# dhillon24/3d-shape-generation

Hardware: AMD Instinct MI355X
Metric: denoising-steps/sec (whole node), 2048-pt DDPM, batch 64 (higher is better)
Workload: dtype f16; 1 GPU; BASELINE configs[1]: point-cloud DDPM (sample2), 2048 points, batch 64 per GPU, 1000-step cosine schedule, fp16 operands/fp32 accumulate, random-init synthetic weights, denoiser UNetPointNetLarge; batch_per_gpu=64, points=2048, sampler=ddpm/sample2, backbone=pointnet, launch=eager, rccl_ranks=1

## Files before the change

### 3d-shape-generation_amd/_lib.py

```python
from __future__ import annotations

import ctypes as C
import os
import subprocess
from typing import Optional

_HERE = os.path.dirname(os.path.abspath(__file__))
LIB_PATH = os.path.join(_HERE, "libpcd_hip.so")
ABI_VERSION = 2
CSRC = os.path.join(_HERE, "csrc")

vp = C.c_void_p
i32, i64, u64, f32, sz = C.c_int, C.c_int64, C.c_uint64, C.c_float, C.c_size_t

PCD_UNET_NLIN = 26


class GemmDesc(C.Structure):
    _fields_ = [("a1", vp), ("lda1", i64), ("k1", i32),
                ("a2", vp), ("lda2", i64), ("k2", i32),
                ("w", vp), ("ldw", i64),
                ("bias", vp), ("shape_bias", vp), ("rows_per_shape", i32),
                ("relu", i32), ("m", i32), ("c", i32)]

# ... 141 lines not shown
    "pcd_head3": (i32, [vp, i64, i32, vp, vp, vp, vp]),
    "pcd_pw_chain_enc1": (i32, [vp, i64, i32, vp, vp, i32, vp, vp, vp, vp, vp, vp]),
    "pcd_pw_chain_enc1_hilo": (i32, [vp, i64, i32, vp, vp, i32, vp, vp, vp, vp, vp, vp]),
    "pcd_pw_chain_tail_hilo": (i32, [vp, i64, vp, vp, vp, vp, vp, vp, vp, vp, vp, vp]),
    "pcd_pw_chain_128": (i32, [vp, i64, vp, vp, vp, vp, vp, vp]),
    "pcd_pw_chain_tail": (i32, [vp, i64, vp, vp, vp, vp, vp, vp, vp, vp, vp, vp]),
    "pcd_unet_config": (i32, [i32]),
    "pcd_panel_chain": (i32, [i32, vp, i64, vp, vp, i32, vp, i64, i32, vp]),
    "pcd_panel_chain_dec": (i32, [vp, vp, i64, vp, vp, i32, vp, i64, i32, vp]),
    "pcd_pw_wide_packed_bytes": (sz, [i32]),
    "pcd_pw_wide_pack": (i32, [i32, vp, vp, vp, vp]),
    "pcd_pw_wide_chain": (i32, [i32, vp, vp, i64, vp, vp, vp]),
    "pcd_pw_wide_ends_packed_bytes": (sz, [i32, i32]),
    "pcd_pw_wide_ends_pack": (i32, [i32, i32, vp, vp, vp, vp]),
    "pcd_pw_wide_ends": (i32, [i32, i32, vp, vp, vp, i64, vp, vp, vp, vp]),
    "pcd_conv1x1_supported": (i32, [i32, i32]),
    "pcd_conv1x1_f16": (i32, [vp, i64, i32, vp, i64, vp, i32, i32, vp, vp]),
    "pcd_unet_create": (i32, [C.POINTER(UnetDesc), C.POINTER(vp)]),
    "pcd_unet_destroy": (None, [vp]),
    "pcd_unet_workspace_bytes": (sz, [i32, i32]),
    "pcd_unet_forward": (i32, [vp, vp, i32, i32, vp, i32, vp, vp, sz, vp]),
    "pcd_unet_profile": (i32, [vp, i32]),
    "pcd_unet_profile_read": (i32, [vp, C.POINTER(C.c_double), C.POINTER(i32)]),
    "pcd_unet_tap": (i32, [vp, C.c_char_p, i32, i32, vp, vp, sz, vp]),
    "pcd_unet_capture": (i32, [vp, vp, vp, vp, vp]),
    "pcd_gemm_f32": (i32, [vp, i64, i32, vp, i64, i32, vp, i64, vp, vp, i32, i32, i32, i32, vp, i64, vp]),
    "pcd_gemm_f32_colmax": (i32, [vp, i64, i32, vp, i64, vp, i32, i32, vp, i32, vp]),
    "pcd_unet_f32_create": (i32, [C.POINTER(UnetDesc), C.POINTER(vp)]),
    "pcd_unet_f32_destroy": (None, [vp]),
    "pcd_unet_f32_workspace_bytes": (sz, [i32, i32]),
# ... 253 lines not shown
```

### 3d-shape-generation_amd/csrc/stage_images.h

```cpp
#pragma once
#include "common.h"

namespace pcd {

static __global__ __launch_bounds__(256) void stage_pack_kernel(const half_t* __restrict__ w, int64_t ldw, int row0, int row_limit, int k0, int ntile, int nq,
                                                                char* __restrict__ dst) {
    const int id = blockIdx.x * blockDim.x + threadIdx.x;
    if (id >= ntile * nq * 64) return;
    const int lane = id & 63, tq = id >> 6, t = tq / nq, q = tq - t * nq;
    const int row = row0 + 32 * t + (lane & 31);
    half8 v;
#pragma unroll
    for (int e = 0; e < 8; ++e) v[e] = (half_t)0.f;
    if (row < row_limit) v = *(const half8*)(w + (int64_t)row * ldw + k0 + 16 * q + 8 * (lane >> 5));
    *(half8*)(dst + (size_t)id * 16) = v;
}

struct FragBlock { int w, ldw, row0, row_limit, k0, ntile, nq, nimg; size_t off; };
struct ParamRow { int src, src_off, n, off; };
struct StageLayout {
    int nblock, nrow;
    size_t par;
    size_t bytes;
    FragBlock block[20];
    ParamRow row[8];
};
constexpr void sl_frag(StageLayout& L, int w, int ldw, int row0, int row_limit, int k0, int ntile, int nq, int nimg = 1) {
    L.block[L.nblock++] = FragBlock{w, ldw, row0, row_limit, k0, ntile, nq, nimg, L.bytes};
    L.bytes += (size_t)nimg * ntile * nq * 1024;
    L.par = L.bytes;
}
constexpr void sl_row(StageLayout& L, int src, int src_off, int n, int width) {
    L.row[L.nrow++] = ParamRow{src, src_off, n, (int)((L.bytes - L.par) / sizeof(float))};
    L.bytes += width * sizeof(float);
}

static inline int stage_pack(const StageLayout& L, const void* const* weights, const float* const* params, void* packed, hipStream_t s) {
    char* dst = (char*)packed;
    PCD_CHECK_HIP(hipMemsetAsync(dst, 0, L.bytes, s));
    for (int i = 0; i < L.nblock; ++i) {
// ... 34 lines not shown
```

### 3d-shape-generation_amd/csrc/unet.hip

```cpp
#include <string.h>
#include <new>
#include "common.h"

struct pcd_unet {
    pcd_unet_desc_t d;
    static constexpr int kMaxEv = 4096;
    int prof_on = 0;
    int prof_n = 0;
    hipEvent_t ev0[kMaxEv];
    hipEvent_t ev1[kMaxEv];
    int ev_created = 0;
    void* wide[2] = {nullptr, nullptr};
    void* ends[2] = {nullptr, nullptr};
    void* gf3_frag = nullptr;
    void* lin_frag[PCD_UNET_NLIN] = {};
    void* dec_tap[4] = {nullptr, nullptr, nullptr, nullptr};
};

namespace pcd {

int pw_chain_enc1_impl(const float* x, int64_t m, int rows_per_shape, const float* w_xyz, const float* tbias, int tbias_shape_stride,
                       const void* w_conv2, const float* b_conv2, const void* w_conv3, const float* b_conv3, void* x1, bool hilo,
                       float* zero, int64_t zero_n, void* stream);


struct UnetWs {
    size_t x1, x2, x3, x4, s0, s1, pooled, pooled16, gbias, total;
};
// ... 16 lines not shown
    return w;
}

}

using namespace pcd;

static const int kLinK[PCD_UNET_NLIN] = {64, 64, 128, 128, 128, 256, 256, 256, 512, 512, 512, 1024, 2048,
                                         1024, 1024, 1024, 1024, 512, 512, 512, 256, 256, 256, 128, 128, 64};
static const int kLinC[PCD_UNET_NLIN] = {64, 128, 128, 128, 256, 256, 256, 512, 512, 512, 1024, 2048, 4096,
                                         1024, 1024, 512, 512, 512, 256, 256, 256, 128, 128, 128, 64, 64};

static int g_unet_chains = 3;

extern "C" int pcd_unet_config(int use_chains) {
    g_unet_chains = use_chains & 15;
    return PCD_OK;
}

extern "C" int pcd_unet_create(const pcd_unet_desc_t* desc, pcd_unet_t** out) {
    PCD_CHECK_ARG(desc != nullptr && out != nullptr);
    PCD_CHECK_ARG(desc->freqs && desc->tw0 && desc->tb0 && desc->tw2 && desc->tb2);
    PCD_CHECK_ARG(desc->e1w_xyz && desc->e1w_t && desc->e1b && desc->wg && desc->head_w && desc->head_b);
    PCD_CHECK_ARG(desc->wg_k == 4096 && desc->wg_c == 1024);
    if (desc->hilo_mask & ~PCD_UNET_HILO_ALLOWED) {
        set_error("pcd_unet_create: hilo_mask 0x%x names layers outside 0x%x", desc->hilo_mask, PCD_UNET_HILO_ALLOWED);
        return PCD_ERR_ARG;
    }
    for (int i = 0; i < PCD_UNET_NLIN; ++i) {
        if (desc->lin[i].w == nullptr || desc->lin[i].b == nullptr || desc->lin[i].k != kLinK[i] ||
            desc->lin[i].c != kLinC[i]) {
// ... 20 lines not shown
    }
    h->gf3_frag = pcd_packed_copy(desc->lin[12].w, (size_t)4096 * 2048 * 2,
                                  [&](void* buf) { return pcd_gemm_pack_wfrag(desc->lin[12].w, 2048, 2048, 4096, buf, nullptr); });
    for (int i = 8; i <= 18; ++i) {
        if (i == 12 || ((desc->hilo_mask >> i) & 1u) || kLinK[i] < 384 || kLinC[i] % 256 != 0) continue;
        h->lin_frag[i] = pcd_packed_copy(desc->lin[i].w, (size_t)kLinK[i] * kLinC[i] * 2,
                                         [&](void* buf) { return pcd_gemm_pack_wfrag(desc->lin[i].w, kLinK[i], kLinK[i], kLinC[i], buf, nullptr); });
    }
    for (int c = 0; c < 2; ++c) {
        const int first = c == 0 ? 2 : 19, nl = c == 0 ? 6 : 4;
        const int hilo = (int)((desc->hilo_mask >> (c == 0 ? 4 : 22)) & 1u);
        const void* w[6]; const float* b[6];
        for (int i = 0; i < nl; ++i) { w[i] = desc->lin[first + i].w; b[i] = desc->lin[first + i].b; }
        h->ends[c] = pcd_packed_copy(w[0], pcd_pw_wide_ends_packed_bytes(c, hilo), [&](void* buf) { return pcd_pw_wide_ends_pack(c, hilo, w, b, buf, nullptr); });
    }
    *out = h;
    return PCD_OK;
}

extern "C" void pcd_unet_destroy(pcd_unet_t* h) {
    if (h == nullptr) return;
    if (h->gf3_frag) (void)hipFree(h->gf3_frag);
    for (int i = 0; i < PCD_UNET_NLIN; ++i) if (h->lin_frag[i]) (void)hipFree(h->lin_frag[i]);
    for (int k = 0; k < 2; ++k) if (h->wide[k]) (void)hipFree(h->wide[k]);
    for (int k = 0; k < 2; ++k) if (h->ends[k]) (void)hipFree(h->ends[k]);
    for (int i = 0; i < h->ev_created; ++i) { (void)hipEventDestroy(h->ev0[i]); (void)hipEventDestroy(h->ev1[i]); }
    delete h;
}

extern "C" int pcd_unet_profile(pcd_unet_t* h, int enable) {
    PCD_CHECK_ARG(h != nullptr);
    h->prof_on = enable ? 1 : 0;
    h->prof_n = 0;
    return PCD_OK;
}

extern "C" int pcd_unet_profile_read(pcd_unet_t* h, double* total_ms, int* launches) {
    PCD_CHECK_ARG(h && total_ms && launches);
    double tot = 0.0;
    for (int i = 0; i < h->prof_n; ++i) {
// ... 45 lines not shown
        set_error("pcd_unet_forward: workspace %zu < required %zu", workspace_bytes, w.total);
        return PCD_ERR_WORKSPACE;
    }
    char* ws = (char*)workspace;
    void *x1 = ws + w.x1, *x2 = ws + w.x2, *x3 = ws + w.x3, *x4 = ws + w.x4, *s0 = ws + w.s0, *s1 = ws + w.s1;
    float* pooled = (float*)(ws + w.pooled);
    float* gbias = (float*)(ws + w.gbias);
    hipStream_t s = (hipStream_t)stream;
    const pcd_unet_desc_t& d = h->d;
    int rc;
    const bool chains = (g_unet_chains & 1) != 0;
    bool pooled_cleared = false;
    const bool wide = (g_unet_chains & 2) != 0 && m % 256 == 0;
    const bool e23 = wide && h->ends[0] != nullptr;
    const bool d21 = wide && h->ends[1] != nullptr && h->dec_tap[2] == nullptr;
    if (chains) {
        const unsigned e1 = d.hilo_mask & 3u;
        if (e1 == 3u || e1 == 0u) {
            PCD_RUN(pw_chain_enc1_impl(x, m, n_points, d.e1w_xyz, tbias, tbias_shape_stride, d.lin[0].w, d.lin[0].b, d.lin[1].w, d.lin[1].b, x1,
                                   e1 == 3u, pooled, (int64_t)batch * 4096, s));
            pooled_cleared = true;
        } else {
            PCD_RUN(pcd_enc1_xyz(x, m, n_points, d.e1w_xyz, 64, tbias, tbias_shape_stride, s0, s));
            PCD_RUN(run_lin(d, 0, m, s0, nullptr, 0, nullptr, 0, s1, s));
            PCD_RUN(run_lin(d, 1, m, s1, nullptr, 0, nullptr, 0, x1, s));
        }
        if (!e23) PCD_RUN(pcd_pw_chain_128(x1, m, d.lin[2].w, d.lin[2].b, d.lin[3].w, d.lin[3].b, s1, s));
    } else {
        PCD_RUN(pcd_enc1_xyz(x, m, n_points, d.e1w_xyz, 64, tbias, tbias_shape_stride, s0, s));
        PCD_RUN(run_lin(d, 0, m, s0, nullptr, 0, nullptr, 0, s1, s));
        PCD_RUN(run_lin(d, 1, m, s1, nullptr, 0, nullptr, 0, x1, s));
        if (!e23) {
            PCD_RUN(run_lin(d, 2, m, x1, nullptr, 0, nullptr, 0, s0, s));
            PCD_RUN(run_lin(d, 3, m, s0, nullptr, 0, nullptr, 0, s1, s));
        }
    }
    if (e23) {
        PCD_RUN(pcd_pw_wide_ends(0, (int)((d.hilo_mask >> 4) & 1u), x1, nullptr, nullptr, m, h->ends[0], x3, x2, s));
    } else {
        PCD_RUN(run_lin(d, 4, m, s1, nullptr, 0, nullptr, 0, x2, s));
        if (wide) {
            PCD_RUN(pcd_pw_wide_chain(0, x2, nullptr, m, h->wide[0], x3, s));
        } else {
            PCD_RUN(run_lin(d, 5, m, x2, nullptr, 0, nullptr, 0, s0, s));
            PCD_RUN(run_lin(d, 6, m, s0, nullptr, 0, nullptr, 0, s1, s));
            PCD_RUN(run_lin(d, 7, m, s1, nullptr, 0, nullptr, 0, x3, s));
        }
    }
    const bool panel = (g_unet_chains & 6) == 2 && m % 128 == 0;
    auto panel_chain = [&](int chain, int first, int nl, const void* in, void* out, int ld) {
        const void* frag[3]; const float* bias[3];
        for (int i = 0; i < nl; ++i) { frag[i] = h->lin_frag[first + i]; bias[i] = d.lin[first + i].b; }
// ... 56 lines not shown
        void* t = s0; s0 = s1; s1 = t;
    } else {
        PCD_RUN(run_lin(d, 15, m, s0, nullptr, 0, nullptr, 0, s1, s, h->lin_frag[15]));
        TAP(0, s1, 512);
        PCD_RUN(run_lin(d, 16, m, s1, x3, 512, nullptr, 0, s0, s, h->lin_frag[16]));
        if (panel && has_frags(17, 2)) {
            PCD_RUN(panel_chain(1, 17, 2, s0, s1, 256));
            void* t = s0; s0 = s1; s1 = t;
        } else {
            PCD_RUN(run_lin(d, 17, m, s0, nullptr, 0, nullptr, 0, s1, s, h->lin_frag[17]));
            PCD_RUN(run_lin(d, 18, m, s1, nullptr, 0, nullptr, 0, s0, s, h->lin_frag[18]));
        }
    }
    TAP(1, s0, 256);
    void *ta = s0, *tb = s1;
    if (d21) {
        PCD_RUN(pcd_pw_wide_ends(1, (int)((d.hilo_mask >> 22) & 1u), s0, x2, x1, m, h->ends[1], s1, nullptr, s));
        ta = s1; tb = s0;
    } else {
        if (wide) {
            PCD_RUN(pcd_pw_wide_chain(1, s0, x2, m, h->wide[1], s1, s));
        } else {
            PCD_RUN(run_lin(d, 19, m, s0, x2, 256, nullptr, 0, s1, s));
            PCD_RUN(run_lin(d, 20, m, s1, nullptr, 0, nullptr, 0, s0, s));
            PCD_RUN(run_lin(d, 21, m, s0, nullptr, 0, nullptr, 0, s1, s));
        }
        TAP(2, s1, 128);
        PCD_RUN(run_lin(d, 22, m, s1, x1, 128, nullptr, 0, s0, s));
    }
    const unsigned tl = (d.hilo_mask >> 23) & 7u;
// ... 36 lines not shown
```

### 3d-shape-generation_amd/csrc/widechain.hip

```cpp
#include "common.h"
#include "stage_images.h"

namespace pcd {

constexpr int WC_WAVES = 8, WC_THREADS = 64 * WC_WAVES, WC_TILE = 32 * WC_WAVES;
constexpr int WC_STAGE = 32768, WC_RING = 3;
constexpr int WC_MAXSEG = 8;

struct WcSeg {
    int src;
    int cont;
    int finish;
    int coff;
    int cvalid;
    int bias_off;
    int keep_b;
    int linear;
};

struct WcParams {
    const half_t* in1; const half_t* in2;
    const char* wpacked;
    const float* bias;
    const float* ln;
// ... 88 lines not shown
    for (const auto& p : pass[chain]) sl_frag(L, p[0], p[1], p[2], p[3], p[4], 8, 4, 4);
    for (const auto& p : pass[chain]) sl_row(L, p[0], p[2], p[5], 256);
    return L;
}
constexpr StageLayout WC_LAYOUT[2] = {wc_layout(0), wc_layout(1)};

constexpr StageLayout wl_layout(int passes) {
    StageLayout L{};
    for (int i = 0; i < passes; ++i) sl_frag(L, 0, 256, 256 * i, 256 * passes, 0, 8, 4, 4);
    sl_row(L, 0, 0, 256 * passes, 256 * passes);
    for (int i = 1; i < 3; ++i) sl_row(L, i, 0, 256, 256);
    return L;
}
constexpr StageLayout WL_LAYOUT[4] = {wl_layout(1), wl_layout(2), wl_layout(3), wl_layout(4)};

constexpr int WE_MAXSEG = 8;
enum { WE_K128_C128 = 0, WE_K128_C256 = 1, WE_K256_C128 = 2, WE_K256_C256 = 3 };

struct WeSeg {
    int kind;
    int src;
    int cont;
    int finish;
    int coff;
    int bias_off;
};

struct WeSegSrc { int layer; int ldw; int c0; int k0; };
struct WePlan {
    int nseg, nstage, nbias, nlayer;
    WeSeg seg[WE_MAXSEG];
    WeSegSrc from[WE_MAXSEG];
    int layer_c[6], layer_bias[6];
};
constexpr int we_kind_images(int kind) { return kind == WE_K128_C128 ? 1 : (kind == WE_K256_C256 ? 4 : 2); }
constexpr void we_add(WePlan& P, int kind, int src, int cont, int finish, int coff, int layer, int ldw, int c0, int k0) {
    P.seg[P.nseg] = WeSeg{kind, src, cont, finish, coff, P.layer_bias[layer] + c0};
    P.from[P.nseg] = WeSegSrc{layer, ldw, c0, k0};
    P.nstage += we_kind_images(kind);
    ++P.nseg;
}
constexpr WePlan we_plan(int chain, int hilo) {
    WePlan P{};
    if (chain == 0) {
        const int c[6] = {128, 128, 256, 256, 256, 512};
        P.nlayer = 6;
        for (int i = 0; i < 6; ++i) { P.layer_c[i] = c[i]; P.layer_bias[i] = P.nbias; P.nbias += c[i]; }
        we_add(P, WE_K128_C128, 1, 0, 1, 0, 0, 128, 0, 0);
        we_add(P, WE_K128_C128, 0, 0, 1, 0, 1, 128, 0, 0);
        if (hilo) {
            we_add(P, WE_K128_C256, 0, 0, 0, 0, 2, 256, 0, 0);
            we_add(P, WE_K128_C256, 0, 1, 3, 0, 2, 256, 0, 128);
        } else {
            we_add(P, WE_K128_C256, 0, 0, 3, 0, 2, 128, 0, 0);
        }
        we_add(P, WE_K256_C256, 0, 0, 1, 0, 3, 256, 0, 0);
        we_add(P, WE_K256_C256, 0, 0, 1, 0, 4, 256, 0, 0);
        we_add(P, WE_K256_C256, 0, 0, 2, 0, 5, 256, 0, 0);
        we_add(P, WE_K256_C256, 0, 0, 2, 256, 5, 256, 256, 0);
    } else {
        const int c[4] = {256, 256, 128, 128};
        P.nlayer = 4;
        for (int i = 0; i < 4; ++i) { P.layer_c[i] = c[i]; P.layer_bias[i] = P.nbias; P.nbias += c[i]; }
        we_add(P, WE_K256_C256, 1, 0, 0, 0, 0, 512, 0, 0);
        we_add(P, WE_K256_C256, 2, 1, 1, 0, 0, 512, 0, 256);
        we_add(P, WE_K256_C256, 0, 0, 1, 0, 1, 256, 0, 0);
        we_add(P, WE_K256_C128, 0, 0, 1, 0, 2, 256, 0, 0);
        if (hilo) {
            we_add(P, WE_K256_C128, 3, 0, 0, 0, 3, 512, 0, 0);
            we_add(P, WE_K256_C128, 0, 1, 2, 0, 3, 512, 0, 256);
        } else {
            we_add(P, WE_K256_C128, 3, 0, 2, 0, 3, 256, 0, 0);
        }
    }
    return P;
}

struct WeParams {
    const half_t* in1; const half_t* in2; const half_t* in3;
    const char* wpacked;
    const float* bias;
    half_t* out;
    half_t* out2;
    int64_t m;
};

template <int CHAIN, bool HILO, int SG, typename Ring>
__device__ __forceinline__ void we_segments(const WeParams& p, const Ring& ring, int& n, int64_t row0, int lrow, int hh, const float* bias_lds, half8 (&bf)[16],
                                            f32x16 (&acc)[8]) {
    constexpr WePlan P = we_plan(CHAIN, HILO);
    if constexpr (SG < P.nseg) {
        constexpr WeSeg S = P.seg[SG];
        constexpr int K = (S.kind == WE_K128_C128 || S.kind == WE_K128_C256) ? 128 : 256, C = (S.kind == WE_K128_C128 || S.kind == WE_K256_C128) ? 128 : 256;
        constexpr int NT = C / 32, NQ = 32 / NT, NS = K / (16 * NQ);
        auto at = [&row0, &lrow, &hh](auto* base, int ld, int col) { return base + row0 * ld + (unsigned)(lrow * ld + col + 8 * hh); };
        if constexpr (S.src == 1 || S.src == 2) {
            const half_t* row = at(S.src == 1 ? p.in1 : p.in2, K, 0);
#pragma unroll
            for (int s = 0; s < K / 16; ++s) bf[s] = *(const half8*)(row + 16 * s);
        }
        if constexpr (S.src == 3) {
            const half_t* row = at(p.in3, 128, 0);
#pragma unroll
            for (int s = 0; s < 8; ++s) bf[8 + s] = *(const half8*)(row + 16 * s);
        }
        if constexpr (!S.cont) {
#pragma unroll
            for (int t = 0; t < NT; ++t)
#pragma unroll
                for (int e = 0; e < 16; ++e) acc[t][e] = 0.f;
        }
#pragma unroll
        for (int ks = 0; ks < NS; ++ks) {
            asm volatile("" : "+s"(n));
            const char* img = ring.acquire(n);
#pragma unroll
            for (int f0 = 0; f0 < 32; f0 += 8) {
                half8 af[8];
#pragma unroll
                for (int f = f0; f < f0 + 8; ++f) af[f - f0] = *(const half8*)(img + ((f % NT) * NQ + f / NT) * 1024);
#pragma unroll
                for (int f = f0; f < f0 + 8; ++f)
                    acc[f % NT] = __builtin_amdgcn_mfma_f32_32x32x16_f16(af[f - f0], bf[NQ * ks + f / NT], acc[f % NT], 0, 0, 0);
            }
            ++n;
        }
        int boff = S.bias_off;
        asm volatile("" : "+s"(boff));
        const float* bseg = bias_lds + boff;
        if constexpr (S.finish == 1) {
#pragma unroll
            for (int t = 0; t < NT; ++t)
#pragma unroll
                for (int gp = 0; gp < 2; ++gp) bf[2 * t + gp] = regroup_bias_clamp(acc[t], gp, bseg + 32 * t, hh, 0.f);
        } else if constexpr (S.finish == 2) {
            half_t* orow = at(p.out, CHAIN == 0 ? 512 : 128, S.coff);
#pragma unroll
            for (int t = 0; t < NT; ++t)
#pragma unroll
                for (int gp = 0; gp < 2; ++gp) *(half8*)(orow + 32 * t + 16 * gp) = regroup_bias_clamp(acc[t], gp, bseg + 32 * t, hh, 0.f);
        } else if constexpr (S.finish == 3) {
            half_t* orow = at(p.out2, 256, 0);
#pragma unroll
            for (int t = 0; t < NT; ++t)
#pragma unroll
                for (int gp = 0; gp < 2; ++gp) {
                    bf[2 * t + gp] = regroup_bias_clamp(acc[t], gp, bseg + 32 * t, hh, 0.f);
                    *(half8*)(orow + 32 * t + 16 * gp) = bf[2 * t + gp];
                }
        }
        we_segments<CHAIN, HILO, SG + 1>(p, ring, n, row0, lrow, hh, bias_lds, bf, acc);
    }
}

template <int CHAIN, bool HILO, bool SPLIT>
__global__ __launch_bounds__(WC_THREADS, 2) void pw_wide_ends_kernel(WeParams p) {
    extern __shared__ __attribute__((aligned(16))) char wc_smem[];
    constexpr WePlan P = we_plan(CHAIN, HILO);
    const int lane = threadIdx.x & 63;
    const int wave = __builtin_amdgcn_readfirstlane(threadIdx.x >> 6);
    const int pnt = lane & 31, hh = lane >> 5;
    float* bias_lds = (float*)(wc_smem + WC_RING * WC_STAGE);
    for (int i = threadIdx.x; i < P.nbias; i += WC_THREADS) bias_lds[i] = p.bias[i];
    const int64_t ntiles = p.m / WC_TILE;
    const int my_tiles = (int)((ntiles - blockIdx.x + gridDim.x - 1) / gridDim.x);
    const int nstage_seq = P.nstage;
    const int total_stages = my_tiles * nstage_seq;
    const StageRing<WC_STAGE, 4, WC_RING> ring{p.wpacked, wc_smem, total_stages, wave, lane, nstage_seq, SPLIT};
    ring.issue(0);
    ring.issue(1);
    int n = 0;
#pragma unroll 1
    for (int ti = 0; ti < my_tiles; ++ti) {
        const int64_t tile = blockIdx.x + (int64_t)ti * gridDim.x;
        int64_t row0 = tile * WC_TILE;
        asm volatile("" : "+s"(row0));
        half8 bf[16];
        f32x16 acc[8];
        we_segments<CHAIN, HILO, 0>(p, ring, n, row0, wave * 32 + pnt, hh, bias_lds, bf, acc);
    }
}

constexpr StageLayout we_layout(const WePlan& P) {
    StageLayout L{};
    for (int sg = 0; sg < P.nseg; ++sg) {
        const WeSegSrc& f = P.from[sg];
        const int kind = P.seg[sg].kind, nt = (kind == WE_K128_C128 || kind == WE_K256_C128) ? 4 : 8;
        sl_frag(L, f.layer, f.ldw, f.c0, P.layer_c[f.layer], f.k0, nt, 32 / nt, we_kind_images(kind));
    }
    for (int i = 0; i < P.nlayer; ++i) sl_row(L, i, 0, P.layer_c[i], P.layer_c[i]);
    return L;
}
constexpr bool we_layout_ok(int chain, int hilo) {
    const WePlan P = we_plan(chain, hilo);
    const StageLayout L = we_layout(P);
    bool ok = L.par == (size_t)P.nstage * WC_STAGE && L.bytes - L.par == P.nbias * sizeof(float);
    for (int i = 0; i < P.nlayer; ++i) ok = ok && L.row[i].off == P.layer_bias[i];
    return ok;
}
static_assert(we_layout_ok(0, 0) && we_layout_ok(0, 1) && we_layout_ok(1, 0) && we_layout_ok(1, 1), "ends: plan and packed layout disagree");

template <int CHAIN, bool HILO>
static hipError_t we_launch(bool split, hipStream_t s, WeParams& p) {
    constexpr StageLayout L = we_layout(we_plan(CHAIN, HILO));
    p.bias = (const float*)(p.wpacked + L.par);
    return ring_launch<pw_wide_ends_kernel<CHAIN, HILO, false>, pw_wide_ends_kernel<CHAIN, HILO, true>>(p.m / WC_TILE, RING_CAP_CU, WC_THREADS,
                                                                                                        WC_RING * WC_STAGE + L.bytes - L.par, split, s, p);
}

}

using namespace pcd;

static int g_wc_split = 1;
extern "C" int pcd_pw_wide_config(int split) { g_wc_split = split < 0 ? 0 : (split > 2 ? 2 : split); return PCD_OK; }

extern "C" size_t pcd_pw_wide_packed_bytes(int chain) { return (chain == 0 || chain == 1) ? WC_LAYOUT[chain].bytes : 0; }
// ... 63 lines not shown
    return stage_pack(we_layout(P), w, b, packed, (hipStream_t)stream);
}

extern "C" int pcd_pw_wide_ends(int chain, int hilo, const void* in1, const void* in2, const void* in3, int64_t m, const void* packed, void* out, void* out2,
                                void* stream) {
    PCD_CHECK_ARG((chain == 0 || chain == 1) && in1 && packed && out && m > 0 && m % WC_TILE == 0 && m <= 0x7fffffff);
    PCD_CHECK_ARG(chain == 0 ? out2 != nullptr : (in2 != nullptr && in3 != nullptr));
    WeParams p{};
    p.in1 = (const half_t*)in1; p.in2 = (const half_t*)in2; p.in3 = (const half_t*)in3; p.m = m;
    p.wpacked = (const char*)packed;
    p.out = (half_t*)out;
    p.out2 = (half_t*)out2;
    hipStream_t s = (hipStream_t)stream;
    const bool split = g_wc_split != 0;
    hipError_t e;
    if (chain == 0) e = hilo ? we_launch<0, true>(split, s, p) : we_launch<0, false>(split, s, p);
    else e = hilo ? we_launch<1, true>(split, s, p) : we_launch<1, false>(split, s, p);
    PCD_CHECK_HIP(e);
    return PCD_OK;
}
```

### include/pcd_hip.h

```cpp
#ifndef PCD_HIP_H
#define PCD_HIP_H

#include <stddef.h>
#include <stdint.h>

#ifdef __cplusplus
extern "C" {
#endif

#define PCD_OK 0
#define PCD_ERR_ARG (-1)
#define PCD_ERR_HIP (-2)
#define PCD_ERR_WORKSPACE (-3)

#define PCD_ABI_VERSION 2

const char* pcd_last_error(void);
int pcd_abi_version(void);
int pcd_device_check(void);

typedef struct {
    const void* a1; int64_t lda1; int k1;
    const void* a2; int64_t lda2; int k2;
    const void* w;  int64_t ldw;
// ... 128 lines not shown
int pcd_conv1x1_f16(const void* in, int64_t m, int k, const void* w, int64_t ldw, const float* bias, int relu, int c,
                    void* out, void* stream);
int pcd_unet_config(int use_chains);
int pcd_panel_chain(int chain, const void* x, int64_t m, const void* const* frag, const float* const* bias, int hilo, void* out, int64_t ld, int cap,
                    void* stream);
int pcd_panel_chain_dec(const void* x, const void* x3, int64_t m, const void* const* frag, const float* const* bias, int hilo, void* out, int64_t ld,
                        int cap, void* stream);
size_t pcd_pw_wide_packed_bytes(int chain);
int pcd_pw_wide_pack(int chain, const void* const* w, const float* const* b, void* packed, void* stream);
int pcd_pw_wide_chain(int chain, const void* in1, const void* in2, int64_t m, const void* packed, void* out, void* stream);
int pcd_pw_wide_config(int split);
size_t pcd_pw_wide_ends_packed_bytes(int chain, int hilo);
int pcd_pw_wide_ends_pack(int chain, int hilo, const void* const* w, const float* const* b, void* packed, void* stream);
int pcd_pw_wide_ends(int chain, int hilo, const void* in1, const void* in2, const void* in3, int64_t m, const void* packed, void* out, void* out2,
                     void* stream);
size_t pcd_pw_wide_ln_linear_packed_bytes(int passes);
int pcd_pw_wide_ln_linear_pack(const void* w, const float* b, int passes, const float* ln_g, const float* ln_b, void* packed, void* stream);
int pcd_pw_wide_ln_linear_supported(int dim, int64_t rows);
int pcd_pw_wide_ln_linear(const void* packed, int passes, int relu, const void* x, int64_t rows, void* out, void* stream);

typedef struct pcd_unet pcd_unet_t;
int pcd_unet_create(const pcd_unet_desc_t* desc, pcd_unet_t** out);
void pcd_unet_destroy(pcd_unet_t* h);
size_t pcd_unet_workspace_bytes(int batch, int n_points);
int pcd_unet_forward(pcd_unet_t* h, const float* x, int batch, int n_points,
                     const float* tbias, int tbias_shape_stride,
                     float* eps, void* workspace, size_t workspace_bytes, void* stream);
int pcd_unet_profile(pcd_unet_t* h, int enable);
int pcd_unet_profile_read(pcd_unet_t* h, double* total_ms, int* launches);
int pcd_unet_tap(pcd_unet_t* h, const char* name, int batch, int n_points,
// ... 440 lines not shown
```

Measured before the change: 311.6 denoising-steps/sec.

## Fuse encoder stage 1 and decoder tail into wide persistent chain kernels

Extends the persistent wide-chain 'ends' kernel with two new plans. E123 folds the first encoder stage into the encoder chain: the xyz/time-bias input layer and the 64-channel convs now run together with the 128/256/512 layers, and the kernel also zeroes the pooled buffer. D21T folds the decoder's final 128→64→64 layers and the 3-channel head into the decoder-end chain, writing eps directly. This removes several kernel launches and intermediate activation round-trips through HBM, in exchange for more segments per kernel, padded short weight images and extra register pressure.

```diff
diff --git a/3d-shape-generation_amd/_lib.py b/3d-shape-generation_amd/_lib.py
--- a/3d-shape-generation_amd/_lib.py
+++ b/3d-shape-generation_amd/_lib.py
@@ -179,6 +179,10 @@
     "pcd_pw_wide_ends_packed_bytes": (sz, [i32, i32]),
     "pcd_pw_wide_ends_pack": (i32, [i32, i32, vp, vp, vp, vp]),
     "pcd_pw_wide_ends": (i32, [i32, i32, vp, vp, vp, i64, vp, vp, vp, vp]),
+    "pcd_pw_wide_outer_packed_bytes": (sz, [i32, i32]),
+    "pcd_pw_wide_outer_pack": (i32, [i32, i32, vp, vp, vp, vp]),
+    "pcd_pw_wide_e123": (i32, [i32, vp, i64, i32, vp, i32, vp, vp, vp, vp, vp, i64, vp]),
+    "pcd_pw_wide_d21t": (i32, [i32, vp, vp, vp, i64, vp, vp, vp]),
     "pcd_conv1x1_supported": (i32, [i32, i32]),
     "pcd_conv1x1_f16": (i32, [vp, i64, i32, vp, i64, vp, i32, i32, vp, vp]),
     "pcd_unet_create": (i32, [C.POINTER(UnetDesc), C.POINTER(vp)]),
diff --git a/3d-shape-generation_amd/csrc/stage_images.h b/3d-shape-generation_amd/csrc/stage_images.h
--- a/3d-shape-generation_amd/csrc/stage_images.h
+++ b/3d-shape-generation_amd/csrc/stage_images.h
@@ -23,7 +23,7 @@
     size_t par;
     size_t bytes;
     FragBlock block[20];
-    ParamRow row[8];
+    ParamRow row[12];
 };
 constexpr void sl_frag(StageLayout& L, int w, int ldw, int row0, int row_limit, int k0, int ntile, int nq, int nimg = 1) {
     L.block[L.nblock++] = FragBlock{w, ldw, row0, row_limit, k0, ntile, nq, nimg, L.bytes};
diff --git a/3d-shape-generation_amd/csrc/unet.hip b/3d-shape-generation_amd/csrc/unet.hip
--- a/3d-shape-generation_amd/csrc/unet.hip
+++ b/3d-shape-generation_amd/csrc/unet.hip
@@ -12,6 +12,8 @@
     int ev_created = 0;
     void* wide[2] = {nullptr, nullptr};
     void* ends[2] = {nullptr, nullptr};
+    void* outer[2] = {nullptr, nullptr};
+    int outer_hilo[2] = {0, 0};
     void* gf3_frag = nullptr;
     void* lin_frag[PCD_UNET_NLIN] = {};
     void* dec_tap[4] = {nullptr, nullptr, nullptr, nullptr};
@@ -58,7 +60,7 @@
 static int g_unet_chains = 3;
 
 extern "C" int pcd_unet_config(int use_chains) {
-    g_unet_chains = use_chains & 15;
+    g_unet_chains = use_chains & 31;
     return PCD_OK;
 }
 
@@ -109,6 +111,23 @@
         for (int i = 0; i < nl; ++i) { w[i] = desc->lin[first + i].w; b[i] = desc->lin[first + i].b; }
         h->ends[c] = pcd_packed_copy(w[0], pcd_pw_wide_ends_packed_bytes(c, hilo), [&](void* buf) { return pcd_pw_wide_ends_pack(c, hilo, w, b, buf, nullptr); });
     }
+    {
+        const unsigned e1 = desc->hilo_mask & 3u, tl = (desc->hilo_mask >> 23) & 7u;
+        if (e1 == 0u || e1 == 3u) {
+            const int hilo = h->outer_hilo[0] = (int)((desc->hilo_mask >> 4) & 1u) | (e1 == 3u ? 2 : 0);
+            const void* w[8]; const float* b[9];
+            for (int i = 0; i < 8; ++i) { w[i] = desc->lin[i].w; b[i] = desc->lin[i].b; }
+            b[8] = desc->e1w_xyz;
+            h->outer[0] = pcd_packed_copy(w[0], pcd_pw_wide_outer_packed_bytes(0, hilo), [&](void* buf) { return pcd_pw_wide_outer_pack(0, hilo, w, b, buf, nullptr); });
+        }
+        if (tl == 0u || tl == 7u) {
+            const int hilo = h->outer_hilo[1] = (int)((desc->hilo_mask >> 22) & 1u) | (tl == 7u ? 2 : 0);
+            const void* w[7]; const float* b[9];
+            for (int i = 0; i < 7; ++i) { w[i] = desc->lin[19 + i].w; b[i] = desc->lin[19 + i].b; }
+            b[7] = desc->head_w; b[8] = desc->head_b;
+            h->outer[1] = pcd_packed_copy(w[0], pcd_pw_wide_outer_packed_bytes(1, hilo), [&](void* buf) { return pcd_pw_wide_outer_pack(1, hilo, w, b, buf, nullptr); });
+        }
+    }
     *out = h;
     return PCD_OK;
 }
@@ -119,6 +138,7 @@
     for (int i = 0; i < PCD_UNET_NLIN; ++i) if (h->lin_frag[i]) (void)hipFree(h->lin_frag[i]);
     for (int k = 0; k < 2; ++k) if (h->wide[k]) (void)hipFree(h->wide[k]);
     for (int k = 0; k < 2; ++k) if (h->ends[k]) (void)hipFree(h->ends[k]);
+    for (int k = 0; k < 2; ++k) if (h->outer[k]) (void)hipFree(h->outer[k]);
     for (int i = 0; i < h->ev_created; ++i) { (void)hipEventDestroy(h->ev0[i]); (void)hipEventDestroy(h->ev1[i]); }
     delete h;
 }
@@ -194,7 +214,13 @@
     const bool wide = (g_unet_chains & 2) != 0 && m % 256 == 0;
     const bool e23 = wide && h->ends[0] != nullptr;
     const bool d21 = wide && h->ends[1] != nullptr && h->dec_tap[2] == nullptr;
-    if (chains) {
+    const bool outer = chains && (g_unet_chains & 16) == 0;
+    const bool e123 = outer && e23 && h->outer[0] != nullptr && ((uintptr_t)tbias & 15) == 0;
+    const bool d21t = outer && d21 && h->outer[1] != nullptr && h->dec_tap[3] == nullptr;
+    if (e123) {
+        PCD_RUN(pcd_pw_wide_e123(h->outer_hilo[0], x, m, n_points, tbias, tbias_shape_stride, h->outer[0], x1, x2, x3, pooled, (int64_t)batch * 4096, s));
+        pooled_cleared = true;
+    } else if (chains) {
         const unsigned e1 = d.hilo_mask & 3u;
         if (e1 == 3u || e1 == 0u) {
             PCD_RUN(pw_chain_enc1_impl(x, m, n_points, d.e1w_xyz, tbias, tbias_shape_stride, d.lin[0].w, d.lin[0].b, d.lin[1].w, d.lin[1].b, x1,
@@ -215,7 +241,8 @@
             PCD_RUN(run_lin(d, 3, m, s0, nullptr, 0, nullptr, 0, s1, s));
         }
     }
-    if (e23) {
+    if (e123) {
+    } else if (e23) {
         PCD_RUN(pcd_pw_wide_ends(0, (int)((d.hilo_mask >> 4) & 1u), x1, nullptr, nullptr, m, h->ends[0], x3, x2, s));
     } else {
         PCD_RUN(run_lin(d, 4, m, s1, nullptr, 0, nullptr, 0, x2, s));
@@ -302,6 +329,10 @@
     }
     TAP(1, s0, 256);
     void *ta = s0, *tb = s1;
+    if (d21t) {
+        PCD_RUN(pcd_pw_wide_d21t(h->outer_hilo[1], s0, x2, x1, m, h->outer[1], eps, s));
+        return PCD_OK;
+    }
     if (d21) {
         PCD_RUN(pcd_pw_wide_ends(1, (int)((d.hilo_mask >> 22) & 1u), s0, x2, x1, m, h->ends[1], s1, nullptr, s));
         ta = s1; tb = s0;
diff --git a/3d-shape-generation_amd/csrc/widechain.hip b/3d-shape-generation_amd/csrc/widechain.hip
--- a/3d-shape-generation_amd/csrc/widechain.hip
+++ b/3d-shape-generation_amd/csrc/widechain.hip
@@ -126,8 +126,10 @@
 }
 constexpr StageLayout WL_LAYOUT[4] = {wl_layout(1), wl_layout(2), wl_layout(3), wl_layout(4)};
 
-constexpr int WE_MAXSEG = 8;
-enum { WE_K128_C128 = 0, WE_K128_C256 = 1, WE_K256_C128 = 2, WE_K256_C256 = 3 };
+constexpr int WE_MAXSEG = 12, WE_MAXLAYER = 8;
+enum { WE_K128_C128 = 0, WE_K128_C256 = 1, WE_K256_C128 = 2, WE_K256_C256 = 3, WE_K128_C64 = 4, WE_K64_C64 = 5, WE_K64_C128 = 6 };
+constexpr int WE_KIND_KC[7][2] = {{128, 128}, {128, 256}, {256, 128}, {256, 256}, {128, 64}, {64, 64}, {64, 128}};
+enum { WE_E23 = 0, WE_D21 = 1, WE_E123 = 2, WE_D21T = 3 };
 
 struct WeSeg {
     int kind;
@@ -136,6 +138,7 @@
     int finish;
     int coff;
     int bias_off;
+    int fold;
 };
 
 struct WeSegSrc { int layer; int ldw; int c0; int k0; };
@@ -143,46 +146,70 @@
     int nseg, nstage, nbias, nlayer;
     WeSeg seg[WE_MAXSEG];
     WeSegSrc from[WE_MAXSEG];
-    int layer_c[6], layer_bias[6];
+    int layer_c[WE_MAXLAYER], layer_bias[WE_MAXLAYER];
+    int nextra, extra_n[2], extra_off[2];
 };
-constexpr int we_kind_images(int kind) { return kind == WE_K128_C128 ? 1 : (kind == WE_K256_C256 ? 4 : 2); }
-constexpr void we_add(WePlan& P, int kind, int src, int cont, int finish, int coff, int layer, int ldw, int c0, int k0) {
-    P.seg[P.nseg] = WeSeg{kind, src, cont, finish, coff, P.layer_bias[layer] + c0};
+constexpr int we_kind_images(int kind) { return kind == WE_K256_C256 ? 4 : (kind == WE_K128_C256 || kind == WE_K256_C128 ? 2 : 1); }
+constexpr void we_add(WePlan& P, int kind, int src, int cont, int finish, int coff, int layer, int ldw, int c0, int k0, int fold = 0) {
+    P.seg[P.nseg] = WeSeg{kind, src, cont, finish, coff, P.layer_bias[layer] + c0, fold};
     P.from[P.nseg] = WeSegSrc{layer, ldw, c0, k0};
     P.nstage += we_kind_images(kind);
     ++P.nseg;
 }
 constexpr WePlan we_plan(int chain, int hilo) {
     WePlan P{};
-    if (chain == 0) {
-        const int c[6] = {128, 128, 256, 256, 256, 512};
-        P.nlayer = 6;
-        for (int i = 0; i < 6; ++i) { P.layer_c[i] = c[i]; P.layer_bias[i] = P.nbias; P.nbias += c[i]; }
-        we_add(P, WE_K128_C128, 1, 0, 1, 0, 0, 128, 0, 0);
-        we_add(P, WE_K128_C128, 0, 0, 1, 0, 1, 128, 0, 0);
-        if (hilo) {
-            we_add(P, WE_K128_C256, 0, 0, 0, 0, 2, 256, 0, 0);
-            we_add(P, WE_K128_C256, 0, 1, 3, 0, 2, 256, 0, 128);
+    const int narrow = hilo & 1, outer = (hilo >> 1) & 1;
+    auto layers = [&P](const int* c, int n) {
+        P.nlayer = n;
+        for (int i = 0; i < n; ++i) { P.layer_c[i] = c[i]; P.layer_bias[i] = P.nbias; P.nbias += c[i]; }
+    };
+    auto extra = [&P](int n) { P.extra_n[P.nextra] = n; P.extra_off[P.nextra++] = P.nbias; P.nbias += (n + 3) / 4 * 4; };
+    if (chain == WE_E23 || chain == WE_E123) {
+        const int c[8] = {64, 128, 128, 128, 256, 256, 256, 512};
+        const int e = chain == WE_E123 ? 2 : 0;
+        layers(c + 2 - e, 6 + e);
+        if (e) {
+            extra(192);
+            we_add(P, WE_K64_C64, 4, 0, 1, 0, 0, outer ? 128 : 64, 0, 0, outer);
+            we_add(P, WE_K64_C128, 0, 0, 4, 0, 1, outer ? 128 : 64, 0, 0, outer);
+        }
+        we_add(P, WE_K128_C128, e ? 0 : 1, 0, 1, 0, e + 0, 128, 0, 0);
+        we_add(P, WE_K128_C128, 0, 0, 1, 0, e + 1, 128, 0, 0);
+        if (narrow) {
+            we_add(P, WE_K128_C256, 0, 0, 0, 0, e + 2, 256, 0, 0);
+            we_add(P, WE_K128_C256, 0, 1, 3, 0, e + 2, 256, 0, 128);
         } else {
-            we_add(P, WE_K128_C256, 0, 0, 3, 0, 2, 128, 0, 0);
-        }
-        we_add(P, WE_K256_C256, 0, 0, 1, 0, 3, 256, 0, 0);
-        we_add(P, WE_K256_C256, 0, 0, 1, 0, 4, 256, 0, 0);
-        we_add(P, WE_K256_C256, 0, 0, 2, 0, 5, 256, 0, 0);
-        we_add(P, WE_K256_C256, 0, 0, 2, 256, 5, 256, 256, 0);
+            we_add(P, WE_K128_C256, 0, 0, 3, 0, e + 2, 128, 0, 0);
+        }
+        we_add(P, WE_K256_C256, 0, 0, 1, 0, e + 3, 256, 0, 0);
+        we_add(P, WE_K256_C256, 0, 0, 1, 0, e + 4, 256, 0, 0);
+        we_add(P, WE_K256_C256, 0, 0, 2, 0, e + 5, 256, 0, 0);
+        we_add(P, WE_K256_C256, 0, 0, 2, 256, e + 5, 256, 256, 0);
     } else {
-        const int c[4] = {256, 256, 128, 128};
-        P.nlayer = 4;
-        for (int i = 0; i < 4; ++i) { P.layer_c[i] = c[i]; P.layer_bias[i] = P.nbias; P.nbias += c[i]; }
+        const int c[7] = {256, 256, 128, 128, 128, 64, 64};
+        const int tail = chain == WE_D21T;
+        layers(c, tail ? 7 : 4);
         we_add(P, WE_K256_C256, 1, 0, 0, 0, 0, 512, 0, 0);
         we_add(P, WE_K256_C256, 2, 1, 1, 0, 0, 512, 0, 256);
         we_add(P, WE_K256_C256, 0, 0, 1, 0, 1, 256, 0, 0);
         we_add(P, WE_K256_C128, 0, 0, 1, 0, 2, 256, 0, 0);
-        if (hilo) {
+        if (narrow) {
             we_add(P, WE_K256_C128, 3, 0, 0, 0, 3, 512, 0, 0);
-            we_add(P, WE_K256_C128, 0, 1, 2, 0, 3, 512, 0, 256);
+            we_add(P, WE_K256_C128, 0, 1, tail ? 1 : 2, 0, 3, 512, 0, 256);
         } else {
-            we_add(P, WE_K256_C128, 3, 0, 2, 0, 3, 256, 0, 0);
+            we_add(P, WE_K256_C128, 3, 0, tail ? 1 : 2, 0, 3, 256, 0, 0);
+        }
+        if (tail) {
+            extra(192);
+            extra(3);
+            if (outer) {
+                we_add(P, WE_K128_C128, 0, 0, 0, 0, 4, 256, 0, 0);
+                we_add(P, WE_K128_C128, 0, 1, 1, 0, 4, 256, 0, 128);
+            } else {
+                we_add(P, WE_K128_C128, 0, 0, 1, 0, 4, 128, 0, 0);
+            }
+            we_add(P, WE_K128_C64, 0, 0, 1, 0, 5, outer ? 256 : 128, 0, 0, outer);
+            we_add(P, WE_K64_C64, 0, 0, 5, 0, 6, outer ? 128 : 64, 0, 0, outer);
         }
     }
     return P;
@@ -195,16 +222,22 @@
     half_t* out;
     half_t* out2;
     int64_t m;
+    const float* xyz; const float* tbias; int rps, tb_stride;
+    half_t* out3;
+    float* zero; int64_t zero_n;
+    float* out32;
 };
 
-template <int CHAIN, bool HILO, int SG, typename Ring>
+template <int CHAIN, int HILO, int SG, typename Ring>
 __device__ __forceinline__ void we_segments(const WeParams& p, const Ring& ring, int& n, int64_t row0, int lrow, int hh, const float* bias_lds, half8 (&bf)[16],
                                             f32x16 (&acc)[8]) {
     constexpr WePlan P = we_plan(CHAIN, HILO);
     if constexpr (SG < P.nseg) {
         constexpr WeSeg S = P.seg[SG];
-        constexpr int K = (S.kind == WE_K128_C128 || S.kind == WE_K128_C256) ? 128 : 256, C = (S.kind == WE_K128_C128 || S.kind == WE_K256_C128) ? 128 : 256;
-        constexpr int NT = C / 32, NQ = 32 / NT, NS = K / (16 * NQ);
+        constexpr int K = WE_KIND_KC[S.kind][0], C = WE_KIND_KC[S.kind][1];
+        constexpr int NT = C / 32, KB = K / 16;
+        constexpr bool SHORT = NT * KB < 32;
+        constexpr int NQ = SHORT ? KB * (1 + S.fold) : 32 / NT, NS = SHORT ? 1 : KB / NQ, NP = NT * NQ;
         auto at = [&row0, &lrow, &hh](auto* base, int ld, int col) { return base + row0 * ld + (unsigned)(lrow * ld + col + 8 * hh); };
         if constexpr (S.src == 1 || S.src == 2) {
             const half_t* row = at(S.src == 1 ? p.in1 : p.in2, K, 0);
@@ -216,6 +249,29 @@
 #pragma unroll
             for (int s = 0; s < 8; ++s) bf[8 + s] = *(const half8*)(row + 16 * s);
         }
+        if constexpr (S.src == 4) {
+            const float* xp = p.xyz + row0 * 3 + (unsigned)(lrow * 3);
+            const float px = xp[0], py = xp[1], pz = xp[2];
+            const unsigned shape = ((unsigned)row0 + (unsigned)lrow) / (unsigned)p.rps;
+            const float* tb = p.tbias + (int64_t)shape * p.tb_stride * 64 + 8 * hh;
+            int xoff = P.extra_off[0];
+            asm volatile("" : "+s"(xoff));
+            const float* wr = bias_lds + xoff + 24 * hh;
+#pragma unroll
+            for (int s = 0; s < 4; ++s) {
+                const f32x4 t0 = *(const f32x4*)(tb + 16 * s), t1 = *(const f32x4*)(tb + 16 * s + 4);
+                half8 o;
+#pragma unroll
+                for (int e = 0; e < 8; ++e) {
+                    float v = e < 4 ? t0[e & 3] : t1[e & 3];
+                    v = fmaf(wr[(16 * s + e) * 3 + 0], px, v);
+                    v = fmaf(wr[(16 * s + e) * 3 + 1], py, v);
+                    v = fmaf(wr[(16 * s + e) * 3 + 2], pz, v);
+                    o[e] = to_half_sat(fmaxf(v, 0.f));
+                }
+                bf[s] = o;
+            }
+        }
         if constexpr (!S.cont) {
 #pragma unroll
             for (int t = 0; t < NT; ++t)
@@ -227,13 +283,13 @@
             asm volatile("" : "+s"(n));
             const char* img = ring.acquire(n);
 #pragma unroll
-            for (int f0 = 0; f0 < 32; f0 += 8) {
+            for (int f0 = 0; f0 < NP; f0 += 8) {
                 half8 af[8];
 #pragma unroll
                 for (int f = f0; f < f0 + 8; ++f) af[f - f0] = *(const half8*)(img + ((f % NT) * NQ + f / NT) * 1024);
 #pragma unroll
                 for (int f = f0; f < f0 + 8; ++f)
-                    acc[f % NT] = __builtin_amdgcn_mfma_f32_32x32x16_f16(af[f - f0], bf[NQ * ks + f / NT], acc[f % NT], 0, 0, 0);
+                    acc[f % NT] = __builtin_amdgcn_mfma_f32_32x32x16_f16(af[f - f0], bf[(NQ * ks + f / NT) % KB], acc[f % NT], 0, 0, 0);
             }
             ++n;
         }
@@ -246,7 +302,7 @@
 #pragma unroll
                 for (int gp = 0; gp < 2; ++gp) bf[2 * t + gp] = regroup_bias_clamp(acc[t], gp, bseg + 32 * t, hh, 0.f);
         } else if constexpr (S.finish == 2) {
-            half_t* orow = at(p.out, CHAIN == 0 ? 512 : 128, S.coff);
+            half_t* orow = at(p.out, CHAIN == WE_E23 || CHAIN == WE_E123 ? 512 : 128, S.coff);
 #pragma unroll
             for (int t = 0; t < NT; ++t)
 #pragma unroll
@@ -260,12 +316,57 @@
                     bf[2 * t + gp] = regroup_bias_clamp(acc[t], gp, bseg + 32 * t, hh, 0.f);
                     *(half8*)(orow + 32 * t + 16 * gp) = bf[2 * t + gp];
                 }
+        } else if constexpr (S.finish == 4) {
+            half_t* orow = at(p.out3, 128, 0);
+#pragma unroll
+            for (int t = 0; t < NT; ++t)
+#pragma unroll
+                for (int gp = 0; gp < 2; ++gp) {
+                    bf[2 * t + gp] = regroup_bias_clamp(acc[t], gp, bseg + 32 * t, hh, 0.f);
+                    *(half8*)(orow + 32 * t + 16 * gp) = bf[2 * t + gp];
+                }
+        } else if constexpr (S.finish == 5) {
+            half8 ch[8];
+#pragma unroll
+            for (int t = 0; t < NT; ++t)
+#pragma unroll
+                for (int gp = 0; gp < 2; ++gp) {
+                    const u32x4_t v = __builtin_bit_cast(u32x4_t, regroup_bias_clamp(acc[t], gp, bseg + 32 * t, hh, 0.f));
+                    u32x4_t c0, c1;
+#pragma unroll
+                    for (int j = 0; j < 4; ++j) {
+                        unsigned a, b;
+                        swap_halves(v[j], v[j], a, b);
+                        c0[j] = a; c1[j] = b;
+                    }
+                    ch[2 * (2 * t + gp)] = __builtin_bit_cast(half8, c0);
+                    ch[2 * (2 * t + gp) + 1] = __builtin_bit_cast(half8, c1);
+                }
+            int hoff = P.extra_off[0];
+            asm volatile("" : "+s"(hoff));
+            const float* hw = p.bias + hoff;
+            float a0 = 0.f, a1 = 0.f, a2 = 0.f;
+#pragma unroll
+            for (int c8 = 0; c8 < 8; ++c8)
+#pragma unroll
+                for (int e = 0; e < 8; ++e) {
+                    const float f = (float)ch[c8][e];
+                    a0 = fmaf(hw[c8 * 8 + e], f, a0);
+                    a1 = fmaf(hw[64 + c8 * 8 + e], f, a1);
+                    a2 = fmaf(hw[128 + c8 * 8 + e], f, a2);
+                }
+            if (hh == 0) {
+                float* o = p.out32 + row0 * 3 + (unsigned)(lrow * 3);
+                o[0] = a0 + hw[192];
+                o[1] = a1 + hw[193];
+                o[2] = a2 + hw[194];
+            }
         }
         we_segments<CHAIN, HILO, SG + 1>(p, ring, n, row0, lrow, hh, bias_lds, bf, acc);
     }
 }
 
-template <int CHAIN, bool HILO, bool SPLIT>
+template <int CHAIN, int HILO, bool SPLIT>
 __global__ __launch_bounds__(WC_THREADS, 2) void pw_wide_ends_kernel(WeParams p) {
     extern __shared__ __attribute__((aligned(16))) char wc_smem[];
     constexpr WePlan P = we_plan(CHAIN, HILO);
@@ -281,6 +382,11 @@
     const StageRing<WC_STAGE, 4, WC_RING> ring{p.wpacked, wc_smem, total_stages, wave, lane, nstage_seq, SPLIT};
     ring.issue(0);
     ring.issue(1);
+    if constexpr (CHAIN == WE_E123) {
+        const f32x4 z4 = {0.f, 0.f, 0.f, 0.f};
+        for (int64_t i = (int64_t)blockIdx.x * WC_THREADS + threadIdx.x; i < p.zero_n / 4; i += (int64_t)gridDim.x * WC_THREADS) ((f32x4*)p.zero)[i] = z4;
+        __syncthreads();
+    }
     int n = 0;
 #pragma unroll 1
     for (int ti = 0; ti < my_tiles; ++ti) {
@@ -297,10 +403,18 @@
     StageLayout L{};
     for (int sg = 0; sg < P.nseg; ++sg) {
         const WeSegSrc& f = P.from[sg];
-        const int kind = P.seg[sg].kind, nt = (kind == WE_K128_C128 || kind == WE_K256_C128) ? 4 : 8;
-        sl_frag(L, f.layer, f.ldw, f.c0, P.layer_c[f.layer], f.k0, nt, 32 / nt, we_kind_images(kind));
+        const int kind = P.seg[sg].kind, nt = WE_KIND_KC[kind][1] / 32, kb = WE_KIND_KC[kind][0] / 16;
+        if (nt * kb < 32) {
+            const int nq = kb * (1 + P.seg[sg].fold);
+            sl_frag(L, f.layer, f.ldw, f.c0, P.layer_c[f.layer], f.k0, nt, nq, 1);
+            L.bytes += (size_t)(32 - nt * nq) * 1024;
+            L.par = L.bytes;
+        } else {
+            sl_frag(L, f.layer, f.ldw, f.c0, P.layer_c[f.layer], f.k0, nt, 32 / nt, we_kind_images(kind));
+        }
     }
     for (int i = 0; i < P.nlayer; ++i) sl_row(L, i, 0, P.layer_c[i], P.layer_c[i]);
+    for (int j = 0; j < P.nextra; ++j) sl_row(L, P.nlayer + j, 0, P.extra_n[j], (P.extra_n[j] + 3) / 4 * 4);
     return L;
 }
 constexpr bool we_layout_ok(int chain, int hilo) {
@@ -308,11 +422,14 @@
     const StageLayout L = we_layout(P);
     bool ok = L.par == (size_t)P.nstage * WC_STAGE && L.bytes - L.par == P.nbias * sizeof(float);
     for (int i = 0; i < P.nlayer; ++i) ok = ok && L.row[i].off == P.layer_bias[i];
+    for (int j = 0; j < P.nextra; ++j) ok = ok && L.row[P.nlayer + j].off == P.extra_off[j];
     return ok;
 }
 static_assert(we_layout_ok(0, 0) && we_layout_ok(0, 1) && we_layout_ok(1, 0) && we_layout_ok(1, 1), "ends: plan and packed layout disagree");
-
-template <int CHAIN, bool HILO>
+static_assert(we_layout_ok(2, 0) && we_layout_ok(2, 1) && we_layout_ok(2, 2) && we_layout_ok(2, 3), "E123: plan and packed layout disagree");
+static_assert(we_layout_ok(3, 0) && we_layout_ok(3, 1) && we_layout_ok(3, 2) && we_layout_ok(3, 3), "D21T: plan and packed layout disagree");
+
+template <int CHAIN, int HILO>
 static hipError_t we_launch(bool split, hipStream_t s, WeParams& p) {
     constexpr StageLayout L = we_layout(we_plan(CHAIN, HILO));
     p.bias = (const float*)(p.wpacked + L.par);
@@ -406,8 +523,54 @@
     hipStream_t s = (hipStream_t)stream;
     const bool split = g_wc_split != 0;
     hipError_t e;
-    if (chain == 0) e = hilo ? we_launch<0, true>(split, s, p) : we_launch<0, false>(split, s, p);
-    else e = hilo ? we_launch<1, true>(split, s, p) : we_launch<1, false>(split, s, p);
+    if (chain == 0) e = hilo ? we_launch<0, 1>(split, s, p) : we_launch<0, 0>(split, s, p);
+    else e = hilo ? we_launch<1, 1>(split, s, p) : we_launch<1, 0>(split, s, p);
     PCD_CHECK_HIP(e);
     return PCD_OK;
 }
+
+extern "C" size_t pcd_pw_wide_outer_packed_bytes(int which, int hilo) {
+    return (which == 0 || which == 1) && hilo >= 0 && hilo <= 3 ? we_layout(we_plan(which == 0 ? WE_E123 : WE_D21T, hilo)).bytes : 0;
+}
+
+extern "C" int pcd_pw_wide_outer_pack(int which, int hilo, const void* const* w, const float* const* b, void* packed, void* stream) {
+    PCD_CHECK_ARG((which == 0 || which == 1) && hilo >= 0 && hilo <= 3 && w && b && packed);
+    const WePlan P = we_plan(which == 0 ? WE_E123 : WE_D21T, hilo);
+    for (int i = 0; i < P.nlayer; ++i) PCD_CHECK_ARG(w[i] != nullptr);
+    for (int i = 0; i < P.nlayer + P.nextra; ++i) PCD_CHECK_ARG(b[i] != nullptr);
+    return stage_pack(we_layout(P), w, b, packed, (hipStream_t)stream);
+}
+
+template <int CHAIN>
+static hipError_t we_launch_hilo(int hilo, bool split, hipStream_t s, WeParams& p) {
+    switch (hilo) {
+        case 0: return we_launch<CHAIN, 0>(split, s, p);
+        case 1: return we_launch<CHAIN, 1>(split, s, p);
+        case 2: return we_launch<CHAIN, 2>(split, s, p);
+        default: return we_launch<CHAIN, 3>(split, s, p);
+    }
+}
+
+extern "C" int pcd_pw_wide_e123(int hilo, const float* xyz, int64_t m, int rows_per_shape, const float* tbias, int tbias_shape_stride, const void* packed,
+                                void* x1, void* x2, void* x3, float* zero, int64_t zero_n, void* stream) {
+    PCD_CHECK_ARG(hilo >= 0 && hilo <= 3 && xyz && tbias && packed && x1 && x2 && x3 && m > 0 && m % WC_TILE == 0 && m <= 0x7fffffff);
+    PCD_CHECK_ARG(rows_per_shape > 0 && tbias_shape_stride >= 0 && ((uintptr_t)tbias & 15) == 0);
+    PCD_CHECK_ARG(zero == nullptr ? zero_n == 0 : (zero_n >= 0 && zero_n % 4 == 0 && ((uintptr_t)zero & 15) == 0));
+    WeParams p{};
+    p.xyz = xyz; p.tbias = tbias; p.rps = rows_per_shape; p.tb_stride = tbias_shape_stride; p.m = m;
+    p.wpacked = (const char*)packed;
+    p.out = (half_t*)x3; p.out2 = (half_t*)x2; p.out3 = (half_t*)x1;
+    p.zero = zero; p.zero_n = zero_n;
+    PCD_CHECK_HIP(we_launch_hilo<WE_E123>(hilo, g_wc_split != 0, (hipStream_t)stream, p));
+    return PCD_OK;
+}
+
+extern "C" int pcd_pw_wide_d21t(int hilo, const void* in1, const void* in2, const void* in3, int64_t m, const void* packed, float* eps, void* stream) {
+    PCD_CHECK_ARG(hilo >= 0 && hilo <= 3 && in1 && in2 && in3 && packed && eps && m > 0 && m % WC_TILE == 0 && m <= 0x7fffffff);
+    WeParams p{};
+    p.in1 = (const half_t*)in1; p.in2 = (const half_t*)in2; p.in3 = (const half_t*)in3; p.m = m;
+    p.wpacked = (const char*)packed;
+    p.out32 = eps;
+    PCD_CHECK_HIP(we_launch_hilo<WE_D21T>(hilo, g_wc_split != 0, (hipStream_t)stream, p));
+    return PCD_OK;
+}
diff --git a/include/pcd_hip.h b/include/pcd_hip.h
--- a/include/pcd_hip.h
+++ b/include/pcd_hip.h
@@ -166,6 +166,11 @@
 int pcd_pw_wide_ends_pack(int chain, int hilo, const void* const* w, const float* const* b, void* packed, void* stream);
 int pcd_pw_wide_ends(int chain, int hilo, const void* in1, const void* in2, const void* in3, int64_t m, const void* packed, void* out, void* out2,
                      void* stream);
+size_t pcd_pw_wide_outer_packed_bytes(int which, int hilo);
+int pcd_pw_wide_outer_pack(int which, int hilo, const void* const* w, const float* const* b, void* packed, void* stream);
+int pcd_pw_wide_e123(int hilo, const float* xyz, int64_t m, int rows_per_shape, const float* tbias, int tbias_shape_stride, const void* packed, void* x1,
+                     void* x2, void* x3, float* zero, int64_t zero_n, void* stream);
+int pcd_pw_wide_d21t(int hilo, const void* in1, const void* in2, const void* in3, int64_t m, const void* packed, float* eps, void* stream);
 size_t pcd_pw_wide_ln_linear_packed_bytes(int passes);
 int pcd_pw_wide_ln_linear_pack(const void* w, const float* b, int passes, const float* ln_g, const float* ln_b, void* packed, void* stream);
 int pcd_pw_wide_ln_linear_supported(int dim, int64_t rows);
```

After: 313.7 denoising-steps/sec, median of 6. About the same (+0.7%).
